# kirstenmaas/nerf-for-angiography

Hardware: AMD Instinct MI355X
Metric: ray-samples/sec (fwd+bwd) (higher is better)
Workload: dtype f16 (f32 accumulate; first layer split bf16; backward stash kept as bf8)

## Files before the change

### nerf_for_angiography_amd/csrc/afx_api.hip

```cpp
#include <hip/hip_runtime.h>
#include <stdarg.h>
#include <stdlib.h>
#include <stdio.h>
#include <algorithm>
#include <string>
#include <vector>
#include "../../include/afx.h"
#include "afx_internal.h"
#include "afx_kernels_f32.hip"
#include "afx_kernels_bf16.hip"
#include "afx_kernels_grid.hip"
#include "afx_kernels_ingrad.hip"
#include "afx_inst.h"
#include <algorithm>
#include <set>

#ifdef AFX_SINGLE_TU
#define AFX_CHAIN16_HERE AFX_CHAIN16_DEF
#else
#define AFX_CHAIN16_HERE AFX_CHAIN16_DECL
#endif
AFX_CHAIN16_FWD(AFX_CHAIN16_HERE, 64) AFX_CHAIN16_BWD(AFX_CHAIN16_HERE, 64)
AFX_CHAIN16_FWD(AFX_CHAIN16_HERE, 128) AFX_CHAIN16_BWD(AFX_CHAIN16_HERE, 128)
AFX_CHAIN16_FWD(AFX_CHAIN16_HERE, 256) AFX_CHAIN16_BWD(AFX_CHAIN16_HERE, 256)
// ... 521 lines not shown
static int launch_wgrad16_t(afx_ctx* c, const WgradArgs& w, const ReduceArgs& rd, int N, hipStream_t st) {
  {
    const size_t lds = (size_t)4 * (F / 8) * (64 * 16 + 64) + (H16 ? 2 * (64 * 2 + 64 * 4) : 0);
    if (!c->attr_done.count((const void*)k_wgrad_bf16<F, H16>)) {
      HIPCHK(hipFuncSetAttribute((const void*)k_wgrad_bf16<F, H16>, hipFuncAttributeMaxDynamicSharedMemorySize, 160 * 1024));
      c->attr_done.insert((const void*)k_wgrad_bf16<F, H16>);
    }
    ProfScope ps(c, AFX_K_WGRAD, st);
    hipLaunchKernelGGL((k_wgrad_bf16<F, H16>), dim3(w.n_splits, N + (w.enc16 ? 1 + (w.coef_cols > 0 ? 1 : 0) : 0)), dim3(512), lds, st, w);
  }
  if (w.small_groups) hipLaunchKernelGGL(k_small_from_groups<F>, dim3(rd.n_small), dim3(F, 4), 0, st, w);
  else hipLaunchKernelGGL((k_small_grads_bf16<F, H16>), dim3(rd.n_small, F / 64), dim3(256), 0, st, w);
  hipLaunchKernelGGL(k_reduce_w<F>, dim3((F * F + 255) / 256, N + 1), dim3(256), 0, st, rd);
  hipLaunchKernelGGL(k_reduce_b<F>, dim3(1, N + 2), dim3(F), 0, st, rd);
  hipLaunchKernelGGL(k_reduce_small<F>, dim3((unsigned)((F * rd.k0pad + 2 * F + 1 + 63) / 64)), dim3(64, 4), 0, st, rd);
  if (w.coef_cols > 0) hipLaunchKernelGGL(k_reduce_coef<F>, dim3(rd.coef_cols), dim3(F), 0, st, rd);
  HIPCHK(hipGetLastError());
  return AFX_OK;
}

template <int F>
static int launch_wgrad8_t(afx_ctx* c, const WgradArgs& w, const ReduceArgs& rd, int N, hipStream_t st) {
  {
    const size_t lds = (size_t)4 * (2 * (F / 16) * (64 * 16 + 128) + 2 * 64 * 4);
    constexpr bool H6 = AFX_H6;
    for (const void* fn : {(const void*)k_wgrad_s8<F, H6>, (const void*)k_wgrad_s8<F, false>})
      if (!c->attr_done.count(fn)) {
        HIPCHK(hipFuncSetAttribute(fn, hipFuncAttributeMaxDynamicSharedMemorySize, 160 * 1024));
        c->attr_done.insert(fn);
      }
    ProfScope ps(c, AFX_K_WGRAD, st);
    const int extra = w.enc16 ? 1 + (w.coef_cols > 0 ? 1 : 0) : 0;
    if (H6 && extra) {
      hipLaunchKernelGGL((k_wgrad_s8<F, true>), dim3(w.n_splits, N), dim3(512), lds, st, w);
      WgradArgs w1 = w;
      w1.y0 = N;
      hipLaunchKernelGGL((k_wgrad_s8<F, false>), dim3(w.n_splits, extra), dim3(512), lds, st, w1);
    } else hipLaunchKernelGGL((k_wgrad_s8<F, H6>), dim3(w.n_splits, N + extra), dim3(512), lds, st, w);
  }
  hipLaunchKernelGGL(k_small_from_groups<F>, dim3(rd.n_small), dim3(F, 4), 0, st, w);
  if (w.no_sw) hipLaunchKernelGGL(k_wout_stash8<F>, dim3(rd.n_small), dim3(2 * F), 0, st, w);
  {
    const int nwx = (F * F + 255) / 256, nw = nwx * (N + 1), nb = N + 2, ns = (int)((F * rd.k0pad + 2 * F + 1 + 63) / 64);
    hipLaunchKernelGGL(k_reduce_all<F>, dim3((unsigned)(nw + nb + ns)), dim3(256), 0, st, rd, nwx, nw, nb);
  }
  if (w.coef_cols > 0) hipLaunchKernelGGL(k_reduce_coef<F>, dim3(rd.coef_cols), dim3(F), 0, st, rd);
  HIPCHK(hipGetLastError());
// ... 93 lines not shown
                           ray1 - ray0, a.target + ray0, a.inv_n, a.pixel + ray0, (float*)a.dod + ray0);
      rc = launch_chain(c, prec, true, p, st, 2);
    } else rc = launch_chain(c, prec, true, a, st);
    if (rc) return rc;
    if (ig) {
      InGradArgs g = *ig;
      g.stash_dz = (const char*)a.stash_dz; g.graw = a.graw;
      if ((rc = launch_input_grads(c, prec, a, g, t0, t1, TILE, st))) return rc;
    }
    if (!grad_flat) continue;
    WgradArgs w = {};
    w.stash_h = a.stash_h; w.stash_dz = a.stash_dz; w.stash_e = a.stash_e; w.graw = a.graw;
    w.rows = (t1 - t0) * TILE;
    w.stride_rows = (int64_t)rows;
    w.n_hidden = N; w.k0 = c->k0; w.k0pad = k0ld;
    const WgradSplit sp = wgrad_split(w.rows, b16 ? c->n_cu / N : (2 * c->n_cu) / (N + 1), kSplits, kSmallBlocks);
    w.n_splits = (int)sp.splits;
    w.rows_per_split = (int)sp.rows_per_split;
    w.partial = partial; w.partial2 = partial2; w.partial_s = partial_s; w.small_groups = sg ? 1 : 0;
    w.gmax = a.gmax; w.stash_esz = (int)esz; w.gexp = a.gexp; w.hexp = a.hexp; w.enc16 = enc16 ? 1 : 0; w.coef_cols = a.coef_cols;
    w.dod = split ? a.dod : nullptr; w.gpr = a.s_pad / GROUP; w.group0 = t0 * (TILE / GROUP); w.group_ray = goff ? a.group_ray : nullptr;
    w.n_groups_valid = goff ? a.n_total / GROUP : n_rays * (int64_t)(a.s_pad / GROUP);
    w.dsz = dsz;
    ReduceArgs rd = {};
    rd.partial = partial; rd.partial2 = partial2; rd.n_hidden = N; rd.k0 = c->k0; rd.k0pad = k0ld; rd.n_splits = w.n_splits;
    rd.grad = grad_flat; rd.hidden_only = b16 ? 1 : 0; rd.partial_s = partial_s;
    rd.n_small = (int)sp.n_small;
    rd.gmax = a.gmax; rd.scale_shift = s8 ? AFX_S8_JSHIFT : 0; rd.layer0_mfma = enc16 ? 1 : 0;
    rd.w0 = c->coef_params; rd.d_coef = c->d_coef; rd.coef_cols = a.coef_cols;
    rd.dsz = dsz;
    rc = with_width(c, [&](auto f) {
      constexpr int FW = decltype(f)::value;
      if (!b16) return launch_wgrad_t<FW>(c, w, rd, N, st);
      if (s8) return launch_wgrad8_t<FW>(c, w, rd, N, st);
      return h16 ? launch_wgrad16_t<FW, true>(c, w, rd, N, st) : launch_wgrad16_t<FW, false>(c, w, rd, N, st);
    });
    if (rc) return rc;
  }
  return AFX_OK;
}

extern "C" int afx_render_backward(afx_ctx* c, int prec, const void* prepared, const afx_render_args* r,
                                   const float* dL_dpixel, float* grad_flat, void* stream) {
  if (c && r && r->n_rays == 0) return AFX_OK;
  int rc = check_render(c, r, "afx_render_backward");
  if (rc) return rc;
// ... 98 lines not shown

struct StashSet { char *stash_h, *stash_dz, *gexp, *masks, *hexp; float *gpart, *records; int64_t rows; };
static StashSet carve_stash_set(const afx_ctx* c, size_t rows, Carve& w) {
  const size_t F = c->d.width, N = c->d.n_hidden;
  StashSet b;
  b.rows = (int64_t)rows;
  b.stash_h = w.take((N + 1) * rows * F); b.stash_dz = w.take((N + 1) * rows * F);
  b.gexp = w.take(rows * 4); b.gpart = w.take<float>(rows * 4);
  b.masks = w.take((rows / 256) * (N + 1) * c->nt * 1024);
  b.records = w.take<float>((rows / 32) * (3 * F + 8) * 4);
  b.hexp = w.take(N * (rows / 32) * 4);
  return b;
}
struct Wgrad8Scratch { float *partial, *partial2, *partial_s; uint32_t* gmax; };
static Wgrad8Scratch carve_wgrad8_scratch(const afx_ctx* c, Carve& w) {
  const size_t F = c->d.width, N = c->d.n_hidden;
  Wgrad8Scratch p;
  p.partial = w.take<float>((N + 2) * (size_t)kSplits * F * F * 4);
  p.partial2 = w.take<float>((N + 2) * (size_t)kSplits * (F + 4) * 4);
  p.partial_s = w.take<float>((size_t)kSmallBlocks * (F * 16 + 2 * F + 4) * 4);
  p.gmax = w.take<uint32_t>(256);
  return p;
}
static int launch_wgrad8_set(afx_ctx* c, const StashSet& b, const Wgrad8Scratch& p, int64_t rows, int n_small, const int64_t* dsz,
                             float* grad_flat, hipStream_t st) {
  const int N = c->d.n_hidden;
  const WgradSplit sp = wgrad_split(rows, c->n_cu / N, kSplits, kSmallBlocks);
  WgradArgs w = {};
  w.stash_h = (float*)b.stash_h; w.stash_dz = (float*)b.stash_dz; w.graw = (float*)b.gexp; w.gexp = (int32_t*)b.gexp; w.hexp = (uint32_t*)b.hexp;
  w.rows = rows; w.stride_rows = b.rows;
  w.n_hidden = N; w.k0 = c->k0; w.k0pad = 16;
  w.n_splits = (int)sp.splits; w.rows_per_split = (int)sp.rows_per_split;
  w.partial = p.partial; w.partial2 = p.partial2; w.partial_s = p.partial_s; w.small_groups = 1;
  w.gmax = p.gmax; w.stash_esz = 1; w.gpr = 1;
  w.records = b.records; w.no_sw = 1; w.gfull = b.gpart;
  w.dsz = dsz;
  ReduceArgs rd = {};
  rd.partial = p.partial; rd.partial2 = p.partial2; rd.n_hidden = N; rd.k0 = c->k0; rd.k0pad = 16; rd.n_splits = w.n_splits;
  rd.grad = grad_flat; rd.hidden_only = 1; rd.partial_s = p.partial_s; rd.n_small = n_small;
  rd.gmax = p.gmax; rd.scale_shift = AFX_S8_JSHIFT;
  rd.dsz = dsz;
  return with_width(c, [&](auto f) { return launch_wgrad8_t<decltype(f)::value>(c, w, rd, N, st); });
}

struct HierFixed { float *sigA, *tauA, *zf, *sigB, *od_part; Wgrad8Scratch p; };
static HierFixed carve_hier_fixed(const afx_ctx* c, int64_t R, int S, int NF, Carve& w) {
  HierFixed h;
  h.sigA = w.take<float>((size_t)R * S * 4); h.tauA = w.take<float>((size_t)R * S * 4);
  h.zf = w.take<float>((size_t)R * NF * 4); h.sigB = w.take<float>((size_t)R * NF * 4);
  h.od_part = w.take<float>((size_t)R * (size_t)(std::max(s_pad_of(S), s_pad_of(NF)) / GROUP) * 4);
  h.p = carve_wgrad8_scratch(c, w);
  return h;
}
static int64_t hier_max_rays(const afx_ctx* c, int64_t R, int S) {
  return std::min<int64_t>((R + 7) / 8 * 8, stash_max_rows(c, 1, 1) / s_pad_of(S) / 8 * 8);
}
static size_t hier_bytes(const afx_ctx* c, int64_t R, int S, int NF, int64_t nr) {
  Carve w;
  carve_hier_fixed(c, R, S, NF, w);
// ... 48 lines not shown
    a.tile0 = (int)(r0 * sp / 256); a.tile1 = (int)((r1 * sp + 255) / 256);
    a.stash_h = (float*)b.stash_h; a.stash_dz = (float*)b.stash_dz; a.stash_e = nullptr; a.graw = (float*)b.gexp; a.gexp = (int32_t*)b.gexp;
    a.gpart = b.gpart; a.masks = b.masks; a.small_part = b.records; a.stash_rows = b.rows; a.hexp = (uint32_t*)b.hexp;
    return a;
  };
  ChainArgs argsA = base;
  argsA.sigma = sigA; argsA.tau = tauA;
  ChainArgs argsB = base;
  argsB.depth_mode = AFX_DEPTH_PER_RAY_Z; argsB.z = zf; argsB.n_samples = NF; argsB.s_pad = (int)spB; argsB.n_total = R * spB;
  argsB.sigma = sigB; argsB.tau = nullptr;
  for (int64_t r0 = 0; r0 < R; r0 += nr) {
    const int64_t r1 = std::min<int64_t>(r0 + nr, R), n = r1 - r0;
    const ChainArgs a = set_args(argsA, A, r0, r1, spA), b = set_args(argsB, B, r0, r1, spB);
    if ((rc = launch_chain(c, prec, true, a, st, 1))) return rc;
    hipLaunchKernelGGL(k_fine_depths, dim3((unsigned)((n + 63) / 64)), dim3(64), 0, st, r->depth_mode == AFX_DEPTH_PER_RAY_Z ? r->z + r0 * S : r->z,
                       r->depth_mode == AFX_DEPTH_PER_RAY_Z ? 1 : 0, (const float*)nullptr, (const float*)(tauA + r0 * S), u + r0 * NF, n, S, NF,
                       (float*)nullptr, zf + r0 * NF);
    if ((rc = launch_chain(c, prec, true, b, st, 1))) return rc;
    hipLaunchKernelGGL(k_hier_composite, dim3((unsigned)((n + 63) / 64)), dim3(64), 0, st, a, r0, n, (const float*)zf, NF, (const float*)sigA, (const float*)sigB,
                       target, inv_n, r->pixel, A.gpart, (int)spA, B.gpart, (int)spB, z_all);
    HIPCHK(hipMemsetAsync(h.p.gmax, 0, 4, st));
    if ((rc = launch_chain(c, prec, true, a, st, 2))) return rc;
    if ((rc = launch_chain(c, prec, true, b, st, 2))) return rc;
    if ((rc = launch_wgrad8_set(c, A, h.p, (int64_t)(a.tile1 - a.tile0) * 256, kSmallBlocks, nullptr, grad_flat, st))) return rc;
    if ((rc = launch_wgrad8_set(c, B, h.p, (int64_t)(b.tile1 - b.tile0) * 256, kSmallBlocks, nullptr, grad_flat, st))) return rc;
  }
  HIPCHK(hipGetLastError());
  return AFX_OK;
}

extern "C" int afx_mlp_backward(afx_ctx* c, int prec, const void* prepared, const float* pts, int64_t n_pts,
                                const float* d_out, float* grad_flat, void* workspace, size_t workspace_bytes, void* stream) {
  if (!c || !prepared || !pts || !d_out || !grad_flat || !workspace) return fail(AFX_E_INVALID, "afx_mlp_backward: null argument");
  if (check_prec(prec, "afx_mlp_backward")) return AFX_E_INVALID;
  if (n_pts < 0 || n_pts > ((int64_t)1 << 31) - 256) return fail(AFX_E_INVALID, "afx_mlp_backward: n_pts must be < 2^31 per call");
  if (n_pts == 0) return AFX_OK;
  ChainArgs a = {};
  fill_model(c, prec, true, prepared, a);
  a.n_total = n_pts; a.mode = 0; a.pts = pts; a.dod = d_out;
  return run_backward(c, prec, a, 0, (char*)workspace, workspace_bytes, grad_flat, (hipStream_t)stream);
}

static InGradArgs ingrad_args(const afx_ctx* c, int prec, const void* prepared) {
  const PrepLayout L = prep_layout(c, prec);
  InGradArgs g = {};
  g.slab0 = (const char*)prepared + L.slab0_off;
  g.slab0_bytes = L.slab0_bytes;
  g.aux = (const float*)((const char*)prepared + L.small_off) + (size_t)(c->d.n_hidden + 2) * c->d.width + 4;
// ... 920 lines not shown
  a.mode = 1; a.org = m.origins; a.dir = m.dirs; a.poses = nullptr;
  a.depth_mode = 4; a.z = tsp; a.te = tep; a.group_ray = gray;
  a.n_samples = GROUP; a.s_pad = GROUP; a.n_total = std::max<int64_t>(L.g_cap, 1) * GROUP;
  a.fused = 0; a.stash8 = 1; a.coef_cols = 0; a.defer_out = 1; a.dod = nullptr;
  a.od_part = L.od; a.gmax = L.p.gmax;
  a.tile0 = 0; a.tile1 = (int)((a.n_total + tile - 1) / tile);
  a.stash_h = (float*)set.stash_h; a.stash_dz = (float*)set.stash_dz; a.stash_e = nullptr;
  a.graw = (float*)set.gexp; a.gexp = (int32_t*)set.gexp; a.gpart = gpart; a.masks = set.masks;
  a.small_part = set.records; a.stash_rows = set.rows; a.hexp = (uint32_t*)set.hexp;
  a.n_dev = dsz + SZ_NTOTAL;
  a.row_raw = row_raw; a.row_tau = row_tau;
  if ((rc = launch_chain(c, prec, true, a, st, 1))) return rc;
  hipLaunchKernelGGL(k_single_eval_composite, blocks_for(R, 4), dim3(256), 0, st, (const float*)row_raw, (const float*)row_tau, (const float*)ts,
                     (const float*)te, (const int64_t*)offsets, (const int64_t*)goff, R, t->early_stop_eps, t->alpha_thre, t->target, t->inv_n, keep,
                     gpart, counts2, pix);
  HIPCHK(hipGetLastError());
  if ((rc = afx_ray_offsets(counts2, R, off2, goff2, totals + 2, stream))) return rc;
  hipLaunchKernelGGL(k_single_eval_finish, dim3((unsigned)((R + 255) / 256)), dim3(256), 0, st, (const int64_t*)totals, (const float*)pix, R, t->pixel,
                     counts_dev, skip_dev, dsz);
  HIPCHK(hipGetLastError());
  HIPCHK(hipMemsetAsync(L.p.gmax, 0, 4, st));
  a.row_raw = nullptr; a.row_tau = nullptr;
  if ((rc = launch_chain(c, prec, true, a, st, 2))) return rc;
  return launch_wgrad8_set(c, set, L.p, set.rows, (int)wgrad_split(set.rows, splits0, kSplits, kSmallBlocks).n_small, dsz, t->grad_flat, st);
}

struct RenderBufs {
  float *org, *dir;
  int32_t* counts;
  int64_t *offsets, *totals;
  float *ts, *te, *pts, *raw;
  int64_t n_cap;
};
static int carve_render(int32_t ray_mode, int64_t R, int64_t S, Carve& w, RenderBufs& b, const char* who) {
  if (ray_mode != AFX_RAYS_ARRAYS && ray_mode != AFX_RAYS_POSE) return fail(AFX_E_INVALID, "%s: bad ray_mode %d", who, ray_mode);
  if (R < 0 || S < 0) return fail(AFX_E_INVALID, "%s: need n_rays >= 0 and max_steps_per_ray >= 0", who);
  if (R > ((int64_t)1 << 31) - 256 || (S > 0 && R > (((int64_t)1 << 31) - 256) / S))
    return fail(AFX_E_INVALID, "%s: %lld rays x %lld steps exceed afx_mlp_infer's 2^31 - 256 points per call; split the rays", who, (long long)R,
                (long long)S);
  b.n_cap = R * S;
  const size_t pose = ray_mode == AFX_RAYS_POSE ? (size_t)R * 12 : 0, n = (size_t)std::max<int64_t>(b.n_cap, 1);
  b.org = w.take<float>(pose); b.dir = w.take<float>(pose);
  b.counts = w.take<int32_t>((size_t)R * 4); b.offsets = w.take<int64_t>((size_t)(R + 1) * 8); b.totals = w.take<int64_t>(2 * 8);
  b.ts = w.take<float>(n * 4); b.te = w.take<float>(n * 4); b.pts = w.take<float>(n * 12);
  b.raw = w.take<float>(n * 4);
  return AFX_OK;
}
// ... 64 lines not shown
```

### nerf_for_angiography_amd/csrc/afx_internal.h

```cpp
#pragma once
#include <hip/hip_runtime.h>
#include <stdint.h>
#include <stddef.h>
#include <stdio.h>
#include "../../include/afx.h"

namespace afx {

constexpr int TILE = 128;
constexpr int GROUP = 32;

constexpr bool chain_occ2(int nt, int phase) { return phase == 2 && nt <= 4; }
constexpr int chain_tps(int nt, bool bwd, bool x3, int phase = 0) {
  return chain_occ2(nt, phase) ? (nt >= 2 ? 2 : 1) : ((nt >= 4 && !x3 && (!bwd || nt == 4)) ? 4 : (nt >= 2 ? 2 : 1));
}
constexpr uint32_t chain_slab0_bytes(int nk0) { return ((uint32_t)nk0 * 2048u + 4095u) / 4096u * 4096u; }
constexpr uint32_t chain_slot_bytes(int nt, int nk0, bool bwd, bool x3, int phase = 0) {
  const uint32_t s0 = phase == 2 ? 0u : (uint32_t)chain_tps(nt, bwd, x3, phase) * chain_slab0_bytes(nk0);
  const uint32_t sh = (uint32_t)chain_tps(nt, bwd, x3, phase) * (uint32_t)nt * 2048u * (x3 ? 2u : 1u);
  return s0 > sh ? s0 : sh;
}

struct ChainArgs {
  const char* stream_fwd;
// ... 65 lines not shown
  int64_t stride_rows;
  int32_t n_hidden, k0, k0pad;
  int32_t n_splits, rows_per_split;
  float* partial;
  float* partial2;
  int32_t debug;
  float* partial_s;
  int32_t small_groups;
  const uint32_t* gmax;
  int32_t stash_esz;
  const int32_t* gexp;
  int y0;
  const uint32_t* hexp;
  int32_t enc16;
  int32_t coef_cols;
  const float* dod;
  const int32_t* group_ray;
  const float* records;
  int32_t no_sw;
  const float* gfull;
  int32_t gpr;
  int64_t group0;
  int64_t n_groups_valid;
  const int64_t* dsz;
};

struct ReduceArgs {
  const float* partial;
  const float* partial2;
  int32_t n_hidden, k0, k0pad, n_splits;
  int32_t hidden_only;
  int32_t layer0_mfma;
  int32_t n_small;
  const float* partial_s;
  float* grad;
  const uint32_t* gmax;
  int32_t scale_shift;
  const float* w0;
  float* d_coef;
  int32_t coef_cols;
  const int64_t* dsz;
};

enum { SZ_NTOTAL = 0, SZ_ROWS = 1, SZ_SPLITS = 2, SZ_RPS = 3, SZ_SMALL = 4, SZ_GROUPS = 5, SZ_COUNT = 8 };

struct WgradSplit { int64_t splits, rows_per_split, n_small; };
// ... 84 lines not shown
```

### nerf_for_angiography_amd/csrc/afx_kernels_bf16.hip

```cpp
#include <hip/hip_runtime.h>
#include <type_traits>
#include <utility>
#include "afx_internal.h"

typedef short s16x4 __attribute__((ext_vector_type(4)));
typedef short s16x8 __attribute__((ext_vector_type(8)));
typedef short s16x2 __attribute__((ext_vector_type(2)));
typedef unsigned int u32x4 __attribute__((ext_vector_type(4)));
typedef unsigned int u32x2 __attribute__((ext_vector_type(2)));
typedef __bf16 bf16x2_t __attribute__((ext_vector_type(2)));
typedef _Float16 f16x2_t __attribute__((ext_vector_type(2)));
typedef _Float16 f16x8_t __attribute__((ext_vector_type(8)));
typedef float f32x2 __attribute__((ext_vector_type(2)));

__device__ __forceinline__ unsigned pack2(float a, float b) {
  f32x2 v = {a, b};
  return __builtin_bit_cast(unsigned, __builtin_convertvector(v, bf16x2_t));
}
__device__ __forceinline__ float bf_lo(unsigned p) { return __builtin_bit_cast(float, p << 16); }
__device__ __forceinline__ float bf_hi(unsigned p) { return __builtin_bit_cast(float, p & 0xffff0000u); }
__device__ __forceinline__ f32x16 mfma_bf16(u32x4 a, u32x4 b, f32x16 c) {
  return __builtin_amdgcn_mfma_f32_32x32x16_bf16(__builtin_bit_cast(s16x8, a), __builtin_bit_cast(s16x8, b), c, 0, 0, 0);
}
__device__ __forceinline__ unsigned pack2h(float a, float b) {
// ... 673 lines not shown
            const float gh = ldexpf(g[cg], AFX_S8_JSHIFT - eg);
            ghat2[cg] = pack2h(gh, gh);
            if (lane == 0) a.gexp[m[cg] >> 5] = eg;
          }
        }
        const float gs = H16 ? 1.f : g[cg];
#pragma unroll
        for (int t = 0; t < NT; ++t) {
          const unsigned b32 = mask_expand(mk16[((N * NT + t) * NCG + cg) * NTH + tid]);
          const f32x4* wp = (const f32x4*)(wout_perm + (hh * NT + t) * 16);
#pragma unroll
          for (int q = 0; q < 4; ++q) {
            const f32x4 w4 = wp[q];
            dz[cg][t][q >> 1][2 * (q & 1)] = pack2t<H16>(w4[0] * gs, w4[1] * gs) & halfmask(b32, 2 * q);
            dz[cg][t][q >> 1][2 * (q & 1) + 1] = pack2t<H16>(w4[2] * gs, w4[3] * gs) & halfmask(b32, 2 * q + 1);
          }
          asm volatile("" : "+v"(dz[cg][t][0]), "+v"(dz[cg][t][1]));
        }
      }
      unsigned hpos[NCG];
#pragma unroll
      for (int cg = 0; cg < NCG; ++cg)
        hpos[cg] = (__float_as_uint(sp[cg].px) * 0x9E3779B1u) ^ (__float_as_uint(sp[cg].py) * 0x7FEB352Du) ^ (__float_as_uint(sp[cg].pz) * 0x846CA68Bu);
      auto stash_dz_tile = [&](int l, int t, u32x4 (*d)[NT][2]) {
#pragma unroll
        for (int cg = 0; cg < NCG; ++cg) {
          if constexpr (S8) {
            const f16x2_t gh = __builtin_bit_cast(f16x2_t, ghat2[cg]);
            const f16x8_t gh8 = {gh[0], gh[0], gh[0], gh[0], gh[0], gh[0], gh[0], gh[0]};
            const u32x4 x0 = __builtin_bit_cast(u32x4, __builtin_bit_cast(f16x8_t, d[cg][t][0]) * gh8);
            const u32x4 x1 = __builtin_bit_cast(u32x4, __builtin_bit_cast(f16x8_t, d[cg][t][1]) * gh8);
            const unsigned src[8] = {x0[0], x0[1], x0[2], x0[3], x1[0], x1[1], x1[2], x1[3]};
            unsigned h = hpos[cg] ^ ((unsigned)(l * NT + t) * 0x85EBCA77u + (unsigned)hh * 0xC2B2AE3Du);
            h ^= h >> 15; h *= 0x2C1B3C6Du; h ^= h >> 13;
            unsigned r[4] = {0u, 0u, 0u, 0u};
#pragma unroll
            for (int j = 0; j < 16; ++j) {
              const f16x2_t pr = __builtin_bit_cast(f16x2_t, src[j >> 1]);
              r[j >> 2] = sr_bf8(r[j >> 2], pr[j & 1], h, j & 3);
            }
            const u32x4 r8 = {r[0], r[1], r[2], r[3]};
            stash_store((char*)a.stash_dz + (size_t)l * a.stash_rows * F + (so[cg] + (uint32_t)(2 * t) * 512u), r8);
          } else {
#pragma unroll
            for (int s = 0; s < 2; ++s)
              stash_store((char*)a.stash_dz + (size_t)l * a.stash_rows * (F * 2) + (so[cg] + (uint32_t)(4 * t + 2 * s) * 512u), d[cg][t][s]);
          }
        }
      };
      auto bwd_layer = [&](int l, u32x4 (*src)[NT][2], u32x4 (*dst)[NT][2]) {
#pragma unroll
        for (int t = 0; t < NT; ++t) {
          if (t % TPS == 0) stepbase = step_begin(!(SG && l == N && t == 0));
          const u32x4* sl = (const u32x4*)(stepbase + (t % TPS) * SLABT);
          stash_dz_tile(l, t, src);
          f32x16 acc[NCG];
          unsigned mw[NCG];
#pragma unroll
          for (int cg = 0; cg < NCG; ++cg) {
            acc[cg] = (f32x16){0.f};
            mw[cg] = mk16[(((l - 1) * NT + t) * NCG + cg) * NTH + tid];
          }
          rolling_mma(sl, src, acc);
          STAMP(5);
#pragma unroll
          for (int cg = 0; cg < NCG; ++cg) {
            const unsigned b32 = mask_expand(mw[cg]);
#pragma unroll
            for (int q = 0; q < 8; ++q)
              dst[cg][t][q >> 2][q & 3] = pack2t<H16>(acc[cg][2 * q], acc[cg][2 * q + 1]) & halfmask(b32, q);
            asm volatile("" : "+v"(dst[cg][t][0]), "+v"(dst[cg][t][1]));
          }
          STAMP(6);
        }
      };
      constexpr bool PINGPONG = NT >= 8;
      u32x4 dn[NCG][NT][2];
      int l = N;
      if (PINGPONG) for (; l >= 2; l -= 2) {
        bwd_layer(l, dz, dn);
        bwd_layer(l - 1, dn, dz);
      }
      for (; l >= 1; --l) {
        bwd_layer(l, dz, dn);
#pragma unroll
        for (int cg = 0; cg < NCG; ++cg)
#pragma unroll
          for (int t = 0; t < NT; ++t) { dz[cg][t][0] = dn[cg][t][0]; dz[cg][t][1] = dn[cg][t][1]; }
      }
      if constexpr (SG && !ENC) {
#pragma unroll
        for (int cg = 0; cg < NCG; ++cg) {
          float* rec = a.small_part + (size_t)(m[cg] >> 5) * (3 * F + 8);
          float tn, dx, dy, dzz;
          ray_param(a, sp[cg], tn, dx, dy, dzz);
          const float t0 = __shfl(tn, 0);
          const float w1 = H16 ? g[cg] * (tn - t0) : tn - t0;
          const f32x16 dT = __builtin_amdgcn_mfma_f32_32x32x2f32(hh == 0 ? w1 : 0.f, 1.f, (f32x16){0.f}, 0, 0, 0);
          f32x16 gT = {0.f};
          if constexpr (H16) gT = __builtin_amdgcn_mfma_f32_32x32x2f32(hh == 0 ? g[cg] : 0.f, 1.f, (f32x16){0.f}, 0, 0, 0);
#pragma unroll
          for (int t = 0; t < NT; ++t) {
            const f32x16 d = transpose_tile(dz[cg][t]);
            float s0 = 0.f, s1 = 0.f;
#pragma unroll
            for (int r = 0; r < 16; ++r) { s0 = H16 ? fmaf(gT[r], d[r], s0) : s0 + d[r]; s1 = fmaf(dT[r], d[r], s1); }
            s0 += __shfl_xor(s0, 32);
            s1 += __shfl_xor(s1, 32);
            rec[F + hh * F + 32 * t + col] = hh ? s1 : s0;
          }
          if (lane == 0) {
            *(f32x4*)(rec + 3 * F) = (f32x4){sp[cg].px, sp[cg].py, sp[cg].pz, dx};
            *(f32x2*)(rec + 3 * F + 4) = (f32x2){dy, dzz};
          }
        }
      } else {
#pragma unroll
        for (int t = 0; t < NT; ++t) stash_dz_tile(0, t, dz);
      }
    }
  }
  if constexpr (BWD && H16 && !P1) {
    __syncthreads();
    if (tid == 0 && *wg_gmax_p) atomicMax(a.gmax, *wg_gmax_p);
  }
  asm volatile("s_waitcnt vmcnt(0)" ::: "memory");
#ifdef AFX_STAMP
  if (BWD && NW == 8 && F == AFX_STAMP_F && blockIdx.x == 0 && lane == 0)
    for (int i = 0; i < 10; ++i) g_stamps[PHASE][wave][i] += ph[i];
#endif
}

__device__ __forceinline__ int fperm(int p) { return (p & ~12) | ((p & 4) << 1) | ((p & 8) >> 1); }

__device__ __forceinline__ void lds_tr16(s16x4& dst, uint32_t addr, int imm) {
  asm volatile("ds_read_b64_tr_b16 %0, %1 offset:%2" : "=v"(dst) : "v"(addr), "n"(imm) : "memory");
}
template <int F, bool H16 = false>
__global__ void __launch_bounds__(512) k_wgrad_bf16(const WgradArgs a) {
  constexpr int NT = F / 32;
  constexpr int TR = NT >= 2 ? NT / 2 : 1, WR = NT / TR;
  constexpr int TC = NT >= 4 ? NT / 4 : 1, WC = NT / TC;
// ... 119 lines not shown
          for (int r = 0; r < 16; ++r)
            P[(size_t)fperm(32 * (wr * TR + i) + rowperm(r) + 4 * hh) * a.k0pad + 32 * (wc * TC + j) + col] = acc[i][j][r];
        }
  }
  if (has_bias && col == 0 && first <= 0) {
#pragma unroll
    for (int r = 0; r < 16; ++r)
      a.partial2[((size_t)layer * a.n_splits + split) * (F + 4) + fperm(32 * (wr * TR + wc) + rowperm(r) + 4 * hh)] = accb[r];
  }
}

typedef int i32x2 __attribute__((ext_vector_type(2)));
typedef int i32x3 __attribute__((ext_vector_type(3)));
typedef int i32x8 __attribute__((ext_vector_type(8)));
__device__ __forceinline__ void lds_tr6(i32x3& dst, uint32_t addr, int imm) {
  asm volatile("ds_read_b96_tr_b6 %0, %1 offset:%2" : "=v"(dst) : "v"(addr), "n"(imm) : "memory");
}
__device__ __forceinline__ void lds_tr8(i32x2& dst, uint32_t addr, int imm) {
  asm volatile("ds_read_b64_tr_b8 %0, %1 offset:%2" : "=v"(dst) : "v"(addr), "n"(imm) : "memory");
}
__device__ __forceinline__ void lds_rd32(int& dst, uint32_t addr, int imm) {
  asm volatile("ds_read_b32 %0, %1 offset:%2" : "=v"(dst) : "v"(addr), "n"(imm) : "memory");
}

template <int F, bool B6>
__global__ void __launch_bounds__(512) k_wgrad_s8(const WgradArgs a) {
  constexpr int NT = F / 32;
  constexpr int TR = NT >= 2 ? NT / 2 : 1, WR = NT / TR;
  constexpr int TC = NT >= 4 ? NT / 4 : 1, WC = NT / TC;
  constexpr int KB = 64;
  constexpr int NCH = F / 16;
  constexpr int CS = KB * 16 + 128;
  constexpr int IMG = NCH * CS;
  constexpr int NS = 4;
  constexpr int GOFF = NS * 2 * IMG;
  constexpr int PER = 2 * ((NCH + 7) / 8);
  constexpr bool H6 = B6;
  constexpr int XW0 = H6 ? 2 : 1;
  constexpr int HOFF = GOFF + NS * KB * 4;
  static_assert(2 * (NT - 1) * CS + 3 * 128 + 1151 < 65536 && IMG < 65536, "ds offset immediates are 16 bits");
  extern __shared__ __attribute__((aligned(16))) char lds[];
  const int tid = threadIdx.x, lane = tid & 63, col = lane & 31, hh = lane >> 5;
  const int wave = __builtin_amdgcn_readfirstlane(tid >> 6);
  const int first = (int)blockIdx.y + a.y0 - a.n_hidden;
  const int layer = first < 0 ? (int)blockIdx.y + a.y0 + 1 : 0, split = blockIdx.x;
  const int slot = first <= 0 ? layer : a.n_hidden + 1;
  const int E = wgrad_scale_exp(a.gmax);
  const char* A = (const char*)a.stash_dz + (size_t)layer * a.stride_rows * F;
  const char* B = first < 0 ? (const char*)a.stash_h + (size_t)(layer - 1) * a.stride_rows * F
                            : (const char*)a.stash_e + (size_t)first * a.stride_rows * 64;
  const uint32_t* hexp = a.hexp + (size_t)(first < 0 ? layer - 1 : 0) * (size_t)(a.stride_rows >> 5);
  int64_t rows = a.rows, rps = a.rows_per_split;
  int n_splits = a.n_splits;
  if (a.dsz) {
    rows = min(rows, a.dsz[SZ_ROWS]); rps = a.dsz[SZ_RPS]; n_splits = (int)a.dsz[SZ_SPLITS];
    if (split >= n_splits) return;
  }
  int64_t r0 = (int64_t)split * rps;
  int64_t r1 = r0 + rps;
  if (r1 > rows) r1 = rows;
  const int nst = r1 > r0 ? (int)((r1 - r0) / KB) : 0;
  const bool active = wave < WR * WC;
  const int wr = wave / WC, wc = wave % WC;
  const bool has_bias = active && wc < TR;

  f32x16 acc[TR][TC], accb = (f32x16){0.f};
#pragma unroll
  for (int i = 0; i < TR; ++i)
#pragma unroll
    for (int j = 0; j < TC; ++j) acc[i][j] = (f32x16){0.f};
  const i32x8 ones8 = {0x3c3c3c3c, 0x3c3c3c3c, 0x3c3c3c3c, 0x3c3c3c3c, 0x3c3c3c3c, 0x3c3c3c3c, 0x3c3c3c3c, 0x3c3c3c3c};

  auto stage_load = [&](int st) {
    const int buf = st % NS;
    char* dA = lds + buf * 2 * IMG;
    char* dB = dA + IMG;
    const int64_t g0 = (r0 + (int64_t)st * KB) >> 5;
    for (int c = wave; c < NCH; c += 8) {
      const size_t src = ((((size_t)(g0 + hh) * NCH + c) << 5) + col) << 4;
      __builtin_amdgcn_global_load_lds(GPTR(A + src), LPTR(dA + c * CS), 16, 0, 0);
      if constexpr (B6) __builtin_amdgcn_global_load_lds(GPTR(B + (src >> 4) * 12), LPTR(dB + c * CS), 12, 0, 0);
      else if (first < 0) __builtin_amdgcn_global_load_lds(GPTR(B + src), LPTR(dB + c * CS), 16, 0, 0);
      else {
        const size_t srcb = ((((size_t)(g0 + hh) * 4 + (c & 3)) << 5) + col) << 4;
        __builtin_amdgcn_global_load_lds(GPTR(B + srcb), LPTR(dB + (c & 3) * CS), 16, 0, 0);
      }
    }
    if (wave == 0) {
      __builtin_amdgcn_global_load_lds(GPTR(a.gexp + g0 + hh), LPTR(lds + GOFF + buf * (KB * 4)), 4, 0, 0);
      if constexpr (H6) __builtin_amdgcn_global_load_lds(GPTR(hexp + g0 + hh), LPTR(lds + HOFF + buf * (KB * 4)), 4, 0, 0);
    }
  };
  const int g4 = lane >> 4, li = lane & 15;
  const uint32_t lbase = (uint32_t)(uintptr_t)LPTR(lds);
  const uint32_t troff = (uint32_t)((g4 & 1) * CS + (16 * (g4 >> 1) + (li >> 1)) * 16 + 8 * (li & 1));
  const uint32_t offA = troff + (uint32_t)(2 * wr * TR * CS), offB = troff + (uint32_t)(IMG + 2 * wc * TC * CS);
  const uint32_t offB6 = (uint32_t)(IMG + 2 * wc * TC * CS + (g4 & 1) * CS + (32 * (g4 >> 1) + li) * 16);

#pragma unroll
  for (int i = 0; i < NS - 1; ++i)
    if (i < nst) stage_load(i);
  for (int st = 0; st < nst; ++st) {
#ifdef AFX_SAFE_WAITS
    asm volatile("s_waitcnt vmcnt(0)" ::: "memory");
#else
    if (st + NS - 2 < nst) {
      if (wave == 0) asm volatile("s_waitcnt vmcnt(%0)" :: "n"((NS - 2) * (PER + XW0)) : "memory");
      else asm volatile("s_waitcnt vmcnt(%0)" :: "n"((NS - 2) * PER) : "memory");
    } else asm volatile("s_waitcnt vmcnt(0)" ::: "memory");
#endif
    asm volatile("s_waitcnt lgkmcnt(0)\n\ts_barrier" ::: "memory");
    if (st + NS - 1 < nst) stage_load(st + NS - 1);
    if (active) {
      const uint32_t sbase = lbase + (uint32_t)((st % NS) * 2 * IMG);
      i32x2 ax[TR][4], bx[TC][4];
      i32x3 b6[TC][2];
      int eg, hx = 0;
      constexpr bool six = B6;
#pragma unroll
      for (int i = 0; i < TR; ++i)
#pragma unroll
        for (int q = 0; q < 4; ++q) lds_tr8(ax[i][q], sbase + offA, 2 * i * CS + (q >> 1) * 512 + (q & 1) * 128);
      if constexpr (six) {
#pragma unroll
        for (int j = 0; j < TC; ++j)
#pragma unroll
          for (int q = 0; q < 2; ++q) lds_tr6(b6[j][q], sbase + offB6, 2 * j * CS + q * 256);
        lds_rd32(hx, lbase + (uint32_t)(HOFF + (st % NS) * (KB * 4)) + (uint32_t)lane * 4u, 0);
      } else {
#pragma unroll
        for (int j = 0; j < TC; ++j)
#pragma unroll
          for (int q = 0; q < 4; ++q) lds_tr8(bx[j][q], sbase + offB, 2 * j * CS + (q >> 1) * 512 + (q & 1) * 128);
      }
      lds_rd32(eg, lbase + (uint32_t)(GOFF + (st % NS) * (KB * 4)) + (uint32_t)lane * 4u, 0);
// ... 17 lines not shown
          for (int j = 0; j < TC; ++j) {
            const i32x8 bb = {b6[j][0][0], b6[j][0][1], b6[j][0][2], b6[j][1][0], b6[j][1][1], b6[j][1][2], 0, 0};
            const int sb = (int)(((unsigned)hx >> (8 * ((wc * TC + j) >> 1))) & 0xffu);
            acc[i][j] = __builtin_amdgcn_mfma_scale_f32_32x32x64_f8f6f4(a8, bb, acc[i][j], 1, 3, 0, sc, 0, sb);
          }
          if (i == wc) accb = __builtin_amdgcn_mfma_scale_f32_32x32x64_f8f6f4(a8, ones8, accb, 1, 1, 0, sc, 0, 127);
        }
      } else {
        i32x8 b8[TC];
#pragma unroll
        for (int j = 0; j < TC; ++j) b8[j] = (i32x8){bx[j][0][0], bx[j][0][1], bx[j][1][0], bx[j][1][1], bx[j][2][0], bx[j][2][1], bx[j][3][0], bx[j][3][1]};
#pragma unroll
        for (int i = 0; i < TR; ++i) {
          const i32x8 a8 = {ax[i][0][0], ax[i][0][1], ax[i][1][0], ax[i][1][1], ax[i][2][0], ax[i][2][1], ax[i][3][0], ax[i][3][1]};
#pragma unroll
          for (int j = 0; j < TC; ++j)
            acc[i][j] = __builtin_amdgcn_mfma_scale_f32_32x32x64_f8f6f4(a8, b8[j], acc[i][j], 1, 1, 0, sc, 0, 127);
          if (i == wc) accb = __builtin_amdgcn_mfma_scale_f32_32x32x64_f8f6f4(a8, ones8, accb, 1, 1, 0, sc, 0, 127);
        }
      }
    }
  }
  float* P = a.partial + ((size_t)slot * n_splits + split) * F * F;
  if (active && first < 0) {
#pragma unroll
    for (int i = 0; i < TR; ++i)
#pragma unroll
      for (int j = 0; j < TC; ++j)
#pragma unroll
        for (int r = 0; r < 16; ++r)
          P[(size_t)fperm8(32 * (wr * TR + i) + rowperm(r) + 4 * hh) * F + fperm8(32 * (wc * TC + j) + col)] = acc[i][j][r];
  } else if (active) {
#pragma unroll
    for (int i = 0; i < TR; ++i)
#pragma unroll
      for (int j = 0; j < TC; ++j)
        if (wc * TC + j < 2) {
#pragma unroll
          for (int r = 0; r < 16; ++r)
            P[(size_t)fperm8(32 * (wr * TR + i) + rowperm(r) + 4 * hh) * a.k0pad + 32 * (wc * TC + j) + col] = acc[i][j][r];
        }
  }
  if (has_bias && col == 0 && first <= 0) {
#pragma unroll
    for (int r = 0; r < 16; ++r)
      a.partial2[((size_t)layer * n_splits + split) * (F + 4) + fperm8(32 * (wr * TR + wc) + rowperm(r) + 4 * hh)] = accb[r];
// ... 297 lines not shown
```

Measured before the change: 363.1 million.

## Stash last-layer dz as mask bits plus per-row bf8 scale, expand in wgrad

For the last hidden layer under the S8 path, the backward chain no longer stores a full bf8 dz tile. It stores a 2-bit-per-element activation mask plus one bf8 gradient scalar per row. The wgrad kernel loads these compact bits, expands them into bf8 tiles in LDS one stage ahead, and after accumulation multiplies the results by the output-weight vector. This cuts stash write and read bandwidth for that layer, at the cost of extra LDS expansion work, an extra barrier and wait, a larger LDS footprint, and a different rounding path.

```diff
diff --git a/nerf_for_angiography_amd/csrc/afx_api.hip b/nerf_for_angiography_amd/csrc/afx_api.hip
--- a/nerf_for_angiography_amd/csrc/afx_api.hip
+++ b/nerf_for_angiography_amd/csrc/afx_api.hip
@@ -567,7 +567,7 @@
 template <int F>
 static int launch_wgrad8_t(afx_ctx* c, const WgradArgs& w, const ReduceArgs& rd, int N, hipStream_t st) {
   {
-    const size_t lds = (size_t)4 * (2 * (F / 16) * (64 * 16 + 128) + 2 * 64 * 4);
+    const size_t lds = (size_t)4 * (2 * (F / 16) * (64 * 16 + 128) + 2 * 64 * 4 + 2 * (F / 32) * 128 + 256);
     constexpr bool H6 = AFX_H6;
     for (const void* fn : {(const void*)k_wgrad_s8<F, H6>, (const void*)k_wgrad_s8<F, false>})
       if (!c->attr_done.count(fn)) {
@@ -707,6 +707,7 @@
     w.dod = split ? a.dod : nullptr; w.gpr = a.s_pad / GROUP; w.group0 = t0 * (TILE / GROUP); w.group_ray = goff ? a.group_ray : nullptr;
     w.n_groups_valid = goff ? a.n_total / GROUP : n_rays * (int64_t)(a.s_pad / GROUP);
     w.dsz = dsz;
+    w.wout_perm = s8 ? a.small + (size_t)(N + 1) * F : nullptr;
     ReduceArgs rd = {};
     rd.partial = partial; rd.partial2 = partial2; rd.n_hidden = N; rd.k0 = c->k0; rd.k0pad = k0ld; rd.n_splits = w.n_splits;
     rd.grad = grad_flat; rd.hidden_only = b16 ? 1 : 0; rd.partial_s = partial_s;
@@ -851,7 +852,7 @@
   p.gmax = w.take<uint32_t>(256);
   return p;
 }
-static int launch_wgrad8_set(afx_ctx* c, const StashSet& b, const Wgrad8Scratch& p, int64_t rows, int n_small, const int64_t* dsz,
+static int launch_wgrad8_set(afx_ctx* c, const ChainArgs& a, const StashSet& b, const Wgrad8Scratch& p, int64_t rows, int n_small, const int64_t* dsz,
                              float* grad_flat, hipStream_t st) {
   const int N = c->d.n_hidden;
   const WgradSplit sp = wgrad_split(rows, c->n_cu / N, kSplits, kSmallBlocks);
@@ -864,6 +865,7 @@
   w.gmax = p.gmax; w.stash_esz = 1; w.gpr = 1;
   w.records = b.records; w.no_sw = 1; w.gfull = b.gpart;
   w.dsz = dsz;
+  w.wout_perm = a.small + (size_t)(N + 1) * c->d.width;
   ReduceArgs rd = {};
   rd.partial = p.partial; rd.partial2 = p.partial2; rd.n_hidden = N; rd.k0 = c->k0; rd.k0pad = 16; rd.n_splits = w.n_splits;
   rd.grad = grad_flat; rd.hidden_only = 1; rd.partial_s = p.partial_s; rd.n_small = n_small;
@@ -958,8 +960,8 @@
     HIPCHK(hipMemsetAsync(h.p.gmax, 0, 4, st));
     if ((rc = launch_chain(c, prec, true, a, st, 2))) return rc;
     if ((rc = launch_chain(c, prec, true, b, st, 2))) return rc;
-    if ((rc = launch_wgrad8_set(c, A, h.p, (int64_t)(a.tile1 - a.tile0) * 256, kSmallBlocks, nullptr, grad_flat, st))) return rc;
-    if ((rc = launch_wgrad8_set(c, B, h.p, (int64_t)(b.tile1 - b.tile0) * 256, kSmallBlocks, nullptr, grad_flat, st))) return rc;
+    if ((rc = launch_wgrad8_set(c, a, A, h.p, (int64_t)(a.tile1 - a.tile0) * 256, kSmallBlocks, nullptr, grad_flat, st))) return rc;
+    if ((rc = launch_wgrad8_set(c, b, B, h.p, (int64_t)(b.tile1 - b.tile0) * 256, kSmallBlocks, nullptr, grad_flat, st))) return rc;
   }
   HIPCHK(hipGetLastError());
   return AFX_OK;
@@ -1926,7 +1928,7 @@
   HIPCHK(hipMemsetAsync(L.p.gmax, 0, 4, st));
   a.row_raw = nullptr; a.row_tau = nullptr;
   if ((rc = launch_chain(c, prec, true, a, st, 2))) return rc;
-  return launch_wgrad8_set(c, set, L.p, set.rows, (int)wgrad_split(set.rows, splits0, kSplits, kSmallBlocks).n_small, dsz, t->grad_flat, st);
+  return launch_wgrad8_set(c, a, set, L.p, set.rows, (int)wgrad_split(set.rows, splits0, kSplits, kSmallBlocks).n_small, dsz, t->grad_flat, st);
 }
 
 struct RenderBufs {
diff --git a/nerf_for_angiography_amd/csrc/afx_internal.h b/nerf_for_angiography_amd/csrc/afx_internal.h
--- a/nerf_for_angiography_amd/csrc/afx_internal.h
+++ b/nerf_for_angiography_amd/csrc/afx_internal.h
@@ -111,6 +111,7 @@
   int32_t gpr;
   int64_t group0;
   int64_t n_groups_valid;
+  const float* wout_perm;
   const int64_t* dsz;
 };
 
diff --git a/nerf_for_angiography_amd/csrc/afx_kernels_bf16.hip b/nerf_for_angiography_amd/csrc/afx_kernels_bf16.hip
--- a/nerf_for_angiography_amd/csrc/afx_kernels_bf16.hip
+++ b/nerf_for_angiography_amd/csrc/afx_kernels_bf16.hip
@@ -719,12 +719,24 @@
 #pragma unroll
       for (int cg = 0; cg < NCG; ++cg)
         hpos[cg] = (__float_as_uint(sp[cg].px) * 0x9E3779B1u) ^ (__float_as_uint(sp[cg].py) * 0x7FEB352Du) ^ (__float_as_uint(sp[cg].pz) * 0x846CA68Bu);
-      auto stash_dz_tile = [&](int l, int t, u32x4 (*d)[NT][2]) {
+      auto stash_dz_tile = [&](int l, int t, u32x4 (*d)[NT][2], auto last) {
 #pragma unroll
         for (int cg = 0; cg < NCG; ++cg) {
           if constexpr (S8) {
+            if constexpr (decltype(last)::value) {
+              char* pl = (char*)a.stash_dz + (size_t)N * a.stash_rows * F;
+              __builtin_nontemporal_store(mk16[((N * NT + t) * NCG + cg) * NTH + tid],
+                                          (unsigned short*)(pl + ((((m[cg] >> 5) * (uint32_t)NT + (uint32_t)t) << 7) + (uint32_t)lane * 2u)));
+              if (t == NT - 1) {
+                unsigned h = hpos[cg] ^ ((unsigned)(N * NT) * 0x85EBCA77u);
+                h ^= h >> 15; h *= 0x2C1B3C6Du; h ^= h >> 13;
+                const unsigned gb = sr_bf8(0u, __builtin_bit_cast(f16x2_t, ghat2[cg])[0], h, 0);
+                if (hh == 0) *(unsigned char*)(pl + (size_t)a.stash_rows * (F / 8) + m[cg]) = (unsigned char)gb;
+              }
+              continue;
+            } else {
             const f16x2_t gh = __builtin_bit_cast(f16x2_t, ghat2[cg]);
-            const f16x8_t gh8 = {gh[0], gh[0], gh[0], gh[0], gh[0], gh[0], gh[0], gh[0]};
+            const f16x8_t gh8 ={gh[0], gh[0], gh[0], gh[0], gh[0], gh[0], gh[0], gh[0]};
             const u32x4 x0 = __builtin_bit_cast(u32x4, __builtin_bit_cast(f16x8_t, d[cg][t][0]) * gh8);
             const u32x4 x1 = __builtin_bit_cast(u32x4, __builtin_bit_cast(f16x8_t, d[cg][t][1]) * gh8);
             const unsigned src[8] = {x0[0], x0[1], x0[2], x0[3], x1[0], x1[1], x1[2], x1[3]};
@@ -738,6 +750,7 @@
             }
             const u32x4 r8 = {r[0], r[1], r[2], r[3]};
             stash_store((char*)a.stash_dz + (size_t)l * a.stash_rows * F + (so[cg] + (uint32_t)(2 * t) * 512u), r8);
+            }
           } else {
 #pragma unroll
             for (int s = 0; s < 2; ++s)
@@ -745,12 +758,12 @@
           }
         }
       };
-      auto bwd_layer = [&](int l, u32x4 (*src)[NT][2], u32x4 (*dst)[NT][2]) {
+      auto bwd_layer = [&](int l, u32x4 (*src)[NT][2], u32x4 (*dst)[NT][2], auto last) {
 #pragma unroll
         for (int t = 0; t < NT; ++t) {
           if (t % TPS == 0) stepbase = step_begin(!(SG && l == N && t == 0));
           const u32x4* sl = (const u32x4*)(stepbase + (t % TPS) * SLABT);
-          stash_dz_tile(l, t, src);
+          stash_dz_tile(l, t, src, last);
           f32x16 acc[NCG];
           unsigned mw[NCG];
 #pragma unroll
@@ -773,18 +786,43 @@
       };
       constexpr bool PINGPONG = NT >= 8;
       u32x4 dn[NCG][NT][2];
+      constexpr std::false_type inner{};
+      auto copy_back = [&]() {
+#pragma unroll
+        for (int cg = 0; cg < NCG; ++cg)
+#pragma unroll
+          for (int t = 0; t < NT; ++t) { dz[cg][t][0] = dn[cg][t][0]; dz[cg][t][1] = dn[cg][t][1]; }
+      };
       int l = N;
-      if (PINGPONG) for (; l >= 2; l -= 2) {
-        bwd_layer(l, dz, dn);
-        bwd_layer(l - 1, dn, dz);
-      }
-      for (; l >= 1; --l) {
-        bwd_layer(l, dz, dn);
-#pragma unroll
-        for (int cg = 0; cg < NCG; ++cg)
-#pragma unroll
-          for (int t = 0; t < NT; ++t) { dz[cg][t][0] = dn[cg][t][0]; dz[cg][t][1] = dn[cg][t][1]; }
-      }
+      bool in_dz = true;
+      if constexpr (S8) {
+        bwd_layer(N, dz, dn, std::true_type{});
+        l = N - 1;
+        if constexpr (PINGPONG) {
+          in_dz = false;
+          for (; l >= 1; l -= 2) {
+            bwd_layer(l, dn, dz, inner);
+            if (l == 1) { in_dz = true; break; }
+            bwd_layer(l - 1, dz, dn, inner);
+          }
+        } else {
+          copy_back();
+          for (; l >= 1; --l) {
+            bwd_layer(l, dz, dn, inner);
+            copy_back();
+          }
+        }
+      } else {
+        if (PINGPONG) for (; l >= 2; l -= 2) {
+          bwd_layer(l, dz, dn, inner);
+          bwd_layer(l - 1, dn, dz, inner);
+        }
+        for (; l >= 1; --l) {
+          bwd_layer(l, dz, dn, inner);
+          copy_back();
+        }
+      }
+      auto finish = [&](u32x4 (*z0)[NT][2]) {
       if constexpr (SG && !ENC) {
 #pragma unroll
         for (int cg = 0; cg < NCG; ++cg) {
@@ -798,7 +836,7 @@
           if constexpr (H16) gT = __builtin_amdgcn_mfma_f32_32x32x2f32(hh == 0 ? g[cg] : 0.f, 1.f, (f32x16){0.f}, 0, 0, 0);
 #pragma unroll
           for (int t = 0; t < NT; ++t) {
-            const f32x16 d = transpose_tile(dz[cg][t]);
+            const f32x16 d = transpose_tile(z0[cg][t]);
             float s0 = 0.f, s1 = 0.f;
 #pragma unroll
             for (int r = 0; r < 16; ++r) { s0 = H16 ? fmaf(gT[r], d[r], s0) : s0 + d[r]; s1 = fmaf(dT[r], d[r], s1); }
@@ -813,8 +851,13 @@
         }
       } else {
 #pragma unroll
-        for (int t = 0; t < NT; ++t) stash_dz_tile(0, t, dz);
-      }
+        for (int t = 0; t < NT; ++t) stash_dz_tile(0, t, z0, inner);
+      }
+      };
+      if constexpr (S8) {
+        if (PINGPONG && !in_dz) finish(dn);
+        else finish(dz);
+      } else finish(dz);
     }
   }
   if constexpr (BWD && H16 && !P1) {
@@ -980,6 +1023,9 @@
 __device__ __forceinline__ void lds_rd32(int& dst, uint32_t addr, int imm) {
   asm volatile("ds_read_b32 %0, %1 offset:%2" : "=v"(dst) : "v"(addr), "n"(imm) : "memory");
 }
+template <int F> __device__ __forceinline__ int wout_perm_idx(int f) {
+  return ((((f >> 2) & 1) * (F / 32) + (f >> 5)) << 4) + (((f >> 3) & 3) << 2) + (f & 3);
+}
 
 template <int F, bool B6>
 __global__ void __launch_bounds__(512) k_wgrad_s8(const WgradArgs a) {
@@ -996,6 +1042,9 @@
   constexpr bool H6 = B6;
   constexpr int XW0 = H6 ? 2 : 1;
   constexpr int HOFF = GOFF + NS * KB * 4;
+  constexpr int MOFF = HOFF + NS * KB * 4;
+  constexpr int MST = 2 * NT * 128 + 256;
+  constexpr int UNITS = KB * NCH;
   static_assert(2 * (NT - 1) * CS + 3 * 128 + 1151 < 65536 && IMG < 65536, "ds offset immediates are 16 bits");
   extern __shared__ __attribute__((aligned(16))) char lds[];
   const int tid = threadIdx.x, lane = tid & 63, col = lane & 31, hh = lane >> 5;
@@ -1021,6 +1070,8 @@
   const bool active = wave < WR * WC;
   const int wr = wave / WC, wc = wave % WC;
   const bool has_bias = active && wc < TR;
+  const bool bits = first < 0 && layer == a.n_hidden && a.wout_perm != nullptr;
+  const char* GH = A + (size_t)a.stride_rows * (F / 8);
 
   f32x16 acc[TR][TC], accb = (f32x16){0.f};
 #pragma unroll
@@ -1029,6 +1080,12 @@
     for (int j = 0; j < TC; ++j) acc[i][j] = (f32x16){0.f};
   const i32x8 ones8 = {0x3c3c3c3c, 0x3c3c3c3c, 0x3c3c3c3c, 0x3c3c3c3c, 0x3c3c3c3c, 0x3c3c3c3c, 0x3c3c3c3c, 0x3c3c3c3c};
 
+  auto bits_load = [&](int sn, int mslot, int c) {
+    const int64_t row0 = r0 + (int64_t)sn * KB;
+    char* dM = lds + MOFF + mslot * MST;
+    if (c < NT) __builtin_amdgcn_global_load_lds(GPTR(A + (size_t)(row0 >> 5) * (NT * 128) + c * 256 + lane * 4), LPTR(dM + c * 256), 4, 0, 0);
+    else __builtin_amdgcn_global_load_lds(GPTR(GH + row0 + (lane & 15) * 4), LPTR(dM + 2 * NT * 128), 4, 0, 0);
+  };
   auto stage_load = [&](int st) {
     const int buf = st % NS;
     char* dA = lds + buf * 2 * IMG;
@@ -1036,7 +1093,8 @@
     const int64_t g0 = (r0 + (int64_t)st * KB) >> 5;
     for (int c = wave; c < NCH; c += 8) {
       const size_t src = ((((size_t)(g0 + hh) * NCH + c) << 5) + col) << 4;
-      __builtin_amdgcn_global_load_lds(GPTR(A + src), LPTR(dA + c * CS), 16, 0, 0);
+      if (bits) bits_load(st + 1 < nst ? st + 1 : st, (st + 1) % NS, c);
+      else __builtin_amdgcn_global_load_lds(GPTR(A + src), LPTR(dA + c * CS), 16, 0, 0);
       if constexpr (B6) __builtin_amdgcn_global_load_lds(GPTR(B + (src >> 4) * 12), LPTR(dB + c * CS), 12, 0, 0);
       else if (first < 0) __builtin_amdgcn_global_load_lds(GPTR(B + src), LPTR(dB + c * CS), 16, 0, 0);
       else {
@@ -1055,6 +1113,32 @@
   const uint32_t offA = troff + (uint32_t)(2 * wr * TR * CS), offB = troff + (uint32_t)(IMG + 2 * wc * TC * CS);
   const uint32_t offB6 = (uint32_t)(IMG + 2 * wc * TC * CS + (g4 & 1) * CS + (32 * (g4 >> 1) + li) * 16);
 
+  auto expand = [&](int s) {
+    const uint32_t mst = lbase + (uint32_t)(MOFF + (s % NS) * MST), dA = lbase + (uint32_t)((s % NS) * 2 * IMG);
+#pragma unroll
+    for (int k = 0; k < (UNITS + 511) / 512; ++k) {
+      if (UNITS < 512 && wave >= UNITS / 64) break;
+      const int u = tid + 512 * k, r = (u & 31) + 32 * (u / (32 * NCH)), c = (u >> 5) & (NCH - 1);
+      unsigned mw, gb;
+      asm volatile("ds_read_u16 %0, %1" : "=v"(mw) : "v"(mst + 2u * (uint32_t)u) : "memory");
+      asm volatile("ds_read_u8 %0, %1 offset:%2" : "=v"(gb) : "v"(mst + (uint32_t)r), "n"(2 * NT * 128) : "memory");
+      asm volatile("s_waitcnt lgkmcnt(0)" : "+v"(mw), "+v"(gb) :: "memory");
+      const unsigned gb4 = gb * 0x01010101u;
+      u32x4 v;
+#pragma unroll
+      for (int d = 0; d < 4; ++d) {
+        const unsigned z = (mw >> (2 * d)) & 0x0303u;
+        const unsigned m1 = (z | (z << 15)) & 0x01010101u;
+        v[d] = ((m1 << 8) - m1) & gb4;
+      }
+      asm volatile("ds_write_b128 %0, %1" :: "v"(dA + (uint32_t)(c * CS + r * 16)), "v"(v) : "memory");
+    }
+  };
+  if (bits && nst > 0) {
+    for (int c = wave; c < NCH; c += 8) bits_load(0, 0, c);
+    asm volatile("s_waitcnt vmcnt(0)\n\ts_barrier" ::: "memory");
+    expand(0);
+  }
 #pragma unroll
   for (int i = 0; i < NS - 1; ++i)
     if (i < nst) stage_load(i);
@@ -1069,6 +1153,7 @@
 #endif
     asm volatile("s_waitcnt lgkmcnt(0)\n\ts_barrier" ::: "memory");
     if (st + NS - 1 < nst) stage_load(st + NS - 1);
+    if (bits && st + 1 < nst) expand(st + 1);
     if (active) {
       const uint32_t sbase = lbase + (uint32_t)((st % NS) * 2 * IMG);
       i32x2 ax[TR][4], bx[TC][4];
@@ -1132,6 +1217,20 @@
     }
   }
   float* P = a.partial + ((size_t)slot * n_splits + split) * F * F;
+  if (bits && active) {
+#pragma unroll
+    for (int i = 0; i < TR; ++i) {
+      float rs[16];
+#pragma unroll
+      for (int r = 0; r < 16; ++r) rs[r] = a.wout_perm[wout_perm_idx<F>(fperm8(32 * (wr * TR + i) + rowperm(r) + 4 * hh))];
+#pragma unroll
+      for (int r = 0; r < 16; ++r) {
+#pragma unroll
+        for (int j = 0; j < TC; ++j) acc[i][j][r] *= rs[r];
+        if (i == wc) accb[r] *= rs[r];
+      }
+    }
+  }
   if (active && first < 0) {
 #pragma unroll
     for (int i = 0; i < TR; ++i)
```

Result: slower. 342.4 million (-5.7%).
